# microsoft/vision-longformer

Measured on NVIDIA H100. Metric: images/sec ViL-Small 224x224 training, higher is better.
Workload: dtype bf16

## Files before the change

### vision_longformer_b200/csrc/vil_common.cuh

```cuda
#pragma once
#include <cuda_runtime.h>
#include <cuda_bf16.h>
#include <cuda_fp16.h>
#include <stdint.h>
#include "../../include/vil_attn.h"

namespace vil {

struct Geo {
  int B, H, D;
  int nx, ny, w, g, exact, mode;
  int padx, pady, mx, my;
  int Nloc, N, w2;
  int npc;
  int noffs;
  int offR[9], offC[9];
  int has_bias;
  float scale;
  float drop_p, drop_scale;
  uint32_t drop_thresh;
  uint32_t seed_lo, seed_hi, drop_off;
};

inline long long ws_off_delta_g(const Geo& g) { return ((long long)g.B * g.H * g.Nloc + 63) & ~63LL; }
// ... 80 lines not shown
}
__device__ __forceinline__ uint32_t philox_word(const uint4& x, uint32_t w) {
  return w == 0 ? x.x : w == 1 ? x.y : w == 2 ? x.z : x.w;
}
__device__ __forceinline__ bool drop_keep(const Geo& g, uint32_t row, uint32_t col, uint32_t sid) {
  return philox_word(philox(g, col >> 2, row, sid), col & 3) >= g.drop_thresh;
}
__device__ __forceinline__ void drop_keep2(const Geo& g, uint32_t row, uint32_t col, uint32_t sid, bool& k0, bool& k1) {
  const uint4 x = philox(g, col >> 2, row, sid);
  const uint32_t w = col & 3;
  k0 = philox_word(x, w) >= g.drop_thresh;
  const uint32_t u1 = w == 3 ? philox(g, (col >> 2) + 1, row, sid).x : philox_word(x, w + 1);
  k1 = u1 >= g.drop_thresh;
}

__device__ __forceinline__ float warp_sum(float v) {
#pragma unroll
  for (int o = 16; o > 0; o >>= 1) v += __shfl_xor_sync(0xffffffffu, v, o);
  return v;
}

}
```

### vision_longformer_b200/csrc/vil_epilogue.cuh

```cuda
#pragma once
#include "vil_common.cuh"

namespace vil {
namespace epi {

constexpr int kWarps = 4;
constexpr int kAnThreads = kWarps * 32;
constexpr int kThreads = 256;

template <typename T> struct Vec4;
template <> struct Vec4<float> {
  static __device__ __forceinline__ void ld(const float* p, float (&r)[4]) {
    const float4 v = __ldg(reinterpret_cast<const float4*>(p)); r[0] = v.x; r[1] = v.y; r[2] = v.z; r[3] = v.w;
  }
  static __device__ __forceinline__ void st(float* p, const float (&r)[4]) {
    *reinterpret_cast<float4*>(p) = make_float4(r[0], r[1], r[2], r[3]);
  }
};
template <> struct Vec4<__nv_bfloat16> {
  static __device__ __forceinline__ void ld(const __nv_bfloat16* p, float (&r)[4]) {
    const uint2 raw = __ldg(reinterpret_cast<const uint2*>(p));
    const float2 a = __bfloat1622float2(*reinterpret_cast<const __nv_bfloat162*>(&raw.x));
    const float2 b = __bfloat1622float2(*reinterpret_cast<const __nv_bfloat162*>(&raw.y));
    r[0] = a.x; r[1] = a.y; r[2] = b.x; r[3] = b.y;
// ... 237 lines not shown
  float t = 0.f;
  if (col < K * C)
    for (int p = py; p < nparts; p += 8) t += partial[(long long)p * K * C + col];
  sm[py][threadIdx.x & 31] = t;
  __syncthreads();
  if (py == 0 && col < K * C) {
    float r = 0.f;
#pragma unroll
    for (int k = 0; k < 8; ++k) r += sm[k][threadIdx.x & 31];
    const int seg = col / C;
    float* o = seg == 0 ? o0 : (seg == 1 ? o1 : o2);
    if (o != nullptr) o[col - seg * C] = r;
  }
}

__device__ __forceinline__ float ex2_approx(float x) { float y; asm("ex2.approx.ftz.f32 %0, %1;" : "=f"(y) : "f"(x)); return y; }
__device__ __forceinline__ float rcp_approx(float x) { float y; asm("rcp.approx.ftz.f32 %0, %1;" : "=f"(y) : "f"(x)); return y; }
struct GeluTerms { float half_erfc_neg; float gauss; };
__device__ __forceinline__ GeluTerms gelu_terms(float u) {
  const float ax = fabsf(u) * 0.70710678118654752f;
  const float e = ex2_approx(-0.72134752044448170f * u * u);
  const float t = rcp_approx(fmaf(0.3275911f, ax, 1.f));
  float pl = fmaf(1.061405429f, t, -1.453152027f);
  pl = fmaf(pl, t, 1.421413741f);
  pl = fmaf(pl, t, -0.284496736f);
  pl = fmaf(pl, t, 0.254829592f);
  const float q = 0.5f * pl * t * e;
  GeluTerms r;
  r.half_erfc_neg = u >= 0.f ? 1.f - q : q;
  r.gauss = e;
  return r;
// ... 134 lines not shown
```

### vision_longformer_b200/csrc/vil_simt.cuh

```cuda
#pragma once
#include "vil_common.cuh"

namespace vil {

template <int HD> struct Tile {
  static constexpr int HH = HD / 2;
  static constexpr int HS = HD + 8;
  static __device__ __forceinline__ int off(int half) { return half * (HH + 4); }
};

struct ChunkId { int b, h, R, C, piece; };

__device__ __forceinline__ ChunkId decode_block(const Geo& g, int bid) {
  ChunkId c;
  c.piece = bid % g.npc; bid /= g.npc;
  c.C = bid % g.my; bid /= g.my;
  c.R = bid % g.mx; bid /= g.mx;
  c.h = bid % g.H;
  c.b = bid / g.H;
  return c;
}

template <typename T, int HD, bool DROP = false>
__global__ void __launch_bounds__(128)
// ... 90 lines not shown
      sp += __shfl_xor_sync(0xffffffffu, sp, 1);
      float bias = 0.f; bool ok = qvalid;
      if (f == 2) {
        if (geo.has_bias) bias = g2l[((long long)geo.H + h) * geo.g + kvr[j]];
      } else {
        const int dr = qr - kvr[j], dc = qc - kvc[j];
        if (geo.exact == 1 && (abs(dr) > w || abs(dc) > w)) ok = false;
        if (geo.has_bias && ok) bias = tab[(dr + 2 * w - 1) * tw + dc + 2 * w - 1];
      }
      if (ok) {
        const float s = fmaf(geo.scale, sp, bias);
        const float* vd = Vs + j * HS + TL::off(half);
        if constexpr (DROP) {
          const float km = drop_keep(geo, drow, (uint32_t)(cbase + j), dsid) ? 1.f : 0.f;
          if (s > m) {
            const float corr = __expf(m - s);
            lsum = lsum * corr + 1.f;
#pragma unroll
            for (int i = 0; i < HH; ++i) oh[i] = fmaf(oh[i], corr, km * vd[i]);
            m = s;
          } else {
            const float p = __expf(s - m);
            lsum += p;
#pragma unroll
            for (int i = 0; i < HH; ++i) oh[i] = fmaf(p * km, vd[i], oh[i]);
          }
        } else {
          if (s > m) {
            const float corr = __expf(m - s);
            lsum = lsum * corr + 1.f;
#pragma unroll
            for (int i = 0; i < HH; ++i) oh[i] = fmaf(oh[i], corr, vd[i]);
            m = s;
          } else {
            const float p = __expf(s - m);
            lsum += p;
#pragma unroll
            for (int i = 0; i < HH; ++i) oh[i] = fmaf(p, vd[i], oh[i]);
          }
        }
      }
    }
  }
  if (qvalid) {
    const float inv = (lsum > 0.f ? 1.f / lsum : 0.f) * (DROP ? geo.drop_scale : 1.f);
#pragma unroll
    for (int i = 0; i < HH; ++i) oh[i] *= inv;
    const long long tokq = (long long)r * geo.ny + c;
    store_seg<T, HH>(row_ptr_w<T>(o, b, h, tokq), half * HH, D, oh);
    if (half == 0) lse[((long long)b * geo.H + h) * geo.Nloc + tokq] = m + logf(lsum);
// ... 38 lines not shown
  for (int i = 0; i < 8; ++i) oacc[i] = 0.f;
  const float bl = geo.has_bias ? g2l[(long long)h * geo.g + a] : 0.f;
  for (int base = row0 + warp * RPW; base < row1; base += ROWS) {
    const int j = base + rw;
    const bool valid = j < row1;
    const int jc = valid ? j : row1 - 1;
    float kk[8], vv[8];
    load_seg<T, 8>(row_ptr<T>(kg, b, h, jc), 8 * sub, D, kk);
    load_seg<T, 8>(row_ptr<T>(vg, b, h, jc), 8 * sub, D, vv);
    const float sp = group_sum<LPR>(dot8(q8, kk));
    float bias = bl;
    if (geo.has_bias && jc < geo.g) bias = g2g[((long long)h * geo.g + a) * geo.g + jc];
    const float sc = valid ? fmaf(geo.scale, sp, bias) : -INFINITY;
    const float mn = fmaxf(m, sc);
    if (mn > -INFINITY) {
      const float corr = __expf(m - mn), p = __expf(sc - mn);
      lsum = fmaf(lsum, corr, p);
      float pk = p;
      if constexpr (DROP) {
        if (!drop_keep(geo, (uint32_t)a, (uint32_t)j, 2u * (uint32_t)(b * geo.H + h) + 1u)) pk = 0.f;
      }
#pragma unroll
      for (int i = 0; i < 8; ++i) oacc[i] = fmaf(oacc[i], corr, pk * vv[i]);
      m = mn;
    }
  }
  float mw = m;
#pragma unroll
  for (int o = LPR; o < 32; o <<= 1) mw = fmaxf(mw, __shfl_xor_sync(0xffffffffu, mw, o));
  const float scw = (m == -INFINITY) ? 0.f : __expf(m - mw);
  const float lw = rows_sum<LPR>(lsum * scw);
#pragma unroll
  for (int i = 0; i < 8; ++i) {
    const float x = rows_sum<LPR>(oacc[i] * scw);
    if (rw == 0) red_o[warp][8 * sub + i] = x;
  }
  if (lane == 0) { red_m[warp] = mw; red_l[warp] = lw; }
  __syncthreads();
  if (tid < HD) {
    float M = -INFINITY;
    for (int x = 0; x < 8; ++x) M = fmaxf(M, red_m[x]);
    float L = 0.f, O = 0.f;
    for (int x = 0; x < 8; ++x) {
      const float s2 = (red_m[x] == -INFINITY) ? 0.f : __expf(red_m[x] - M);
      L += red_l[x] * s2; O += red_o[x][tid] * s2;
    }
    if (tid < D) row_ptr_w<TO>(og, b, h, a)[tid] = ElemTraits<TO>::from_f(DROP ? O / L * geo.drop_scale : O / L);
    if (tid == 0) lse_g[((long long)b * geo.H + h) * geo.g + a] = M + logf(L);
  }
}

template <typename T, typename TO = T>
__global__ void simt_bwd_delta(Geo geo, T4 o, T4 d_o, T4 og, T4 d_og,
                               float* __restrict__ delta, float* __restrict__ delta_g) {
  const long long rows_loc = (long long)geo.B * geo.H * geo.Nloc;
  const long long rows = rows_loc + (long long)geo.B * geo.H * geo.g;
  const long long idx = (long long)blockIdx.x * (blockDim.x >> 2) + (threadIdx.x >> 2);
  const int sub = threadIdx.x & 3;
  float acc = 0.f;
// ... 120 lines not shown
      const float* vd = Vs + j * HS + TL::off(half);
      float sp = 0.f, dpp = 0.f;
#pragma unroll
      for (int i = 0; i < HH; ++i) { sp = fmaf(qh[i], kd[i], sp); dpp = fmaf(doh[i], vd[i], dpp); }
      sp += __shfl_xor_sync(0xffffffffu, sp, 1);
      dpp += __shfl_xor_sync(0xffffffffu, dpp, 1);
      float bias = 0.f; bool ok = qvalid; int bidx = -1;
      if (f == 2) {
        if (geo.has_bias) bias = g2l[((long long)geo.H + h) * geo.g + kvr[j]];
      } else {
        const int dr = qr - kvr[j], dc = qc - kvc[j];
        if (geo.exact == 1 && (abs(dr) > w || abs(dc) > w)) ok = false;
        if (geo.has_bias && ok) { bidx = (dr + 2 * w - 1) * tw + dc + 2 * w - 1; bias = tab[bidx]; }
      }
      if (ok) {
        const float p = __expf(fmaf(geo.scale, sp, bias) - lse_i);
        if constexpr (DROP) dpp *= km;
        const float ds = p * (dpp - del_i);
#pragma unroll
        for (int i = 0; i < HH; ++i) dqh[i] = fmaf(ds, kd[i], dqh[i]);
        if (bidx >= 0 && half == 0 && d_table != nullptr)
          atomicAdd(d_table + (long long)bidx * geo.H + h, ds);
      }
    }
  }
  if (qvalid) {
#pragma unroll
    for (int i = 0; i < HH; ++i) dqh[i] *= geo.scale;
    store_seg<T, HH>(row_ptr_w<T>(dq, b, h, tokq), half * HH, D, dqh);
  }
}
// ... 76 lines not shown
      __syncthreads();
      for (int i2 = 0; i2 < 64; ++i2) {
        if (!qfl[i2]) continue;
        const float* qd = Qs + i2 * HS + TL::off(half);
        const float* gd = Gs + i2 * HS + TL::off(half);
        float sp = 0.f, dpp = 0.f;
#pragma unroll
        for (int i = 0; i < HH; ++i) { sp = fmaf(kh[i], qd[i], sp); dpp = fmaf(vh[i], gd[i], dpp); }
        sp += __shfl_xor_sync(0xffffffffu, sp, 1);
        dpp += __shfl_xor_sync(0xffffffffu, dpp, 1);
        const int dr = qrs[i2] - vr, dc = qcs[i2] - vc;
        bool ok = kvis;
        if (geo.exact == 1 && (abs(dr) > w || abs(dc) > w)) ok = false;
        if (ok) {
          const float bias = geo.has_bias ? tab[(dr + 2 * w - 1) * tw + dc + 2 * w - 1] : 0.f;
          float p = __expf(fmaf(geo.scale, sp, bias) - lse_s[i2]);
          if constexpr (DROP) {
            const float km = drop_keep(geo, (uint32_t)qtok[i2], (uint32_t)(geo.g + oi * geo.w2 + lk), 2u * (uint32_t)(b * geo.H + h))
                                 ? geo.drop_scale : 0.f;
            const float ds = p * (dpp * km - del_s[i2]);
            p *= km;
#pragma unroll
            for (int i = 0; i < HH; ++i) { dkh[i] = fmaf(ds, qd[i], dkh[i]); dvh[i] = fmaf(p, gd[i], dvh[i]); }
          } else {
            const float ds = p * (dpp - del_s[i2]);
#pragma unroll
            for (int i = 0; i < HH; ++i) { dkh[i] = fmaf(ds, qd[i], dkh[i]); dvh[i] = fmaf(p, gd[i], dvh[i]); }
          }
        }
      }
    }
// ... 33 lines not shown
  load_seg<T, 8>(row_ptr<T>(v, b, h, t), 8 * sub, D, v8);
  const float bias = geo.has_bias ? g2l[((long long)geo.H + h) * geo.g + t] : 0.f;
  float adk[8], adv[8], adb = 0.f;
#pragma unroll
  for (int i = 0; i < 8; ++i) { adk[i] = 0.f; adv[i] = 0.f; }
  const long long base_l = ((long long)b * geo.H + h) * geo.Nloc;
  for (int base = row0 + warp * RPW; base < row1; base += ROWS) {
    const int i2 = base + rw;
    const bool valid = i2 < row1;
    const int ic = valid ? i2 : row1 - 1;
    float qq[8], gg[8];
    load_seg<T, 8>(row_ptr<T>(q, b, h, ic), 8 * sub, D, qq);
    load_seg<T, 8>(row_ptr<T>(d_o, b, h, ic), 8 * sub, D, gg);
    const float ls = lse[base_l + ic], dl = delta[base_l + ic];
    const float sp = group_sum<LPR>(dot8(qq, k8)), dpp = group_sum<LPR>(dot8(gg, v8));
    float p = valid ? __expf(fmaf(geo.scale, sp, bias) - ls) : 0.f;
    float dpk = dpp;
    if constexpr (DROP) {
      const float km = drop_keep(geo, (uint32_t)ic, (uint32_t)t, 2u * (uint32_t)(b * geo.H + h)) ? geo.drop_scale : 0.f;
      dpk = dpp * km;
      const float ds = p * (dpk - dl);
      if (sub == 0) adb += ds;
      p *= km;
#pragma unroll
      for (int i = 0; i < 8; ++i) { adk[i] = fmaf(ds, qq[i], adk[i]); adv[i] = fmaf(p, gg[i], adv[i]); }
    } else {
      const float ds = p * (dpk - dl);
      if (sub == 0) adb += ds;
#pragma unroll
      for (int i = 0; i < 8; ++i) { adk[i] = fmaf(ds, qq[i], adk[i]); adv[i] = fmaf(p, gg[i], adv[i]); }
    }
// ... 44 lines not shown
      const int jc = valid ? j : row1 - 1;
      float kk[8], vv[8], ok_[8], ov_[8];
      load_seg<T, 8>(row_ptr<T>(kg, b, h, jc), 8 * sub, D, kk);
      load_seg<T, 8>(row_ptr<T>(vg, b, h, jc), 8 * sub, D, vv);
      const bool rmw = base < rmw_rows;
      if (add && rmw) {
        load_seg<TO, 8>(row_ptr<TO>(dkg, b, h, jc), 8 * sub, D, ok_);
        load_seg<TO, 8>(row_ptr<TO>(dvg, b, h, jc), 8 * sub, D, ov_);
      } else {
#pragma unroll
        for (int i = 0; i < 8; ++i) { ok_[i] = 0.f; ov_[i] = 0.f; }
      }
      const float sp = group_sum<LPR>(dot8(q8, kk)), dpp = group_sum<LPR>(dot8(g8, vv));
      float bias = bl;
      if (geo.has_bias && jc < geo.g) bias = g2g[((long long)h * geo.g + a) * geo.g + jc];
      const float p = valid ? __expf(fmaf(geo.scale, sp, bias) - lg) : 0.f;
      float km = 1.f;
      if constexpr (DROP) km = drop_keep(geo, (uint32_t)a, (uint32_t)jc, 2u * (uint32_t)(b * geo.H + h) + 1u) ? geo.drop_scale : 0.f;
      const float ds = DROP ? p * (dpp * km - dg) : p * (dpp - dg);
      const float pv = DROP ? p * km : p;
      if (geo.has_bias && valid && sub == 0) {
        if (j < geo.g) { if (d_g2g) atomicAdd(d_g2g + ((long long)h * geo.g + a) * geo.g + j, ds); }
        else adb += ds;
      }
      const float dss = ds * geo.scale;
#pragma unroll
      for (int i = 0; i < 8; ++i) {
        adq[i] = fmaf(ds, kk[i], adq[i]);
        ok_[i] = fmaf(dss, q8[i], ok_[i]);
        ov_[i] = fmaf(pv, g8[i], ov_[i]);
      }
// ... 46 lines not shown
```

### vision_longformer_b200/csrc/vil_wgmma.cuh

```cuda
#pragma once
#include "vil_common.cuh"
#include "vil_sm90.cuh"

namespace vil {
namespace wg {

constexpr int kThreads = 128;

struct Cta { int b, h, R, C, piece; };

__device__ __forceinline__ Cta decode(const Geo& g, int bid) {
  Cta c;
  c.piece = bid % g.npc; bid /= g.npc;
  c.C = bid % g.my; bid /= g.my;
  c.R = bid % g.mx; bid /= g.mx;
  c.h = bid % g.H;
  c.b = bid / g.H;
  return c;
}

__device__ __forceinline__ int acc_row(int i) { return ((threadIdx.x >> 5) << 4) + ((threadIdx.x & 31) >> 2) + (((i >> 1) & 1) << 3); }
__device__ __forceinline__ int acc_col(int i) { return ((i >> 2) << 3) + ((threadIdx.x & 3) << 1) + (i & 1); }

constexpr int kStages = 3;
// ... 43 lines not shown
}

__device__ __forceinline__ void drop_rows(const Geo& geo, int R, int C, int piece, uint32_t (&row)[2]) {
#pragma unroll
  for (int e = 0; e < 2; ++e) {
    const int l = piece * 64 + acc_row(2 * e);
    row[e] = (uint32_t)((R * geo.w + l / geo.w) * geo.ny + C * geo.w + l % geo.w);
  }
}

struct Visit {
  int r, c;
  int dR, dC;
  int cut;
  int oi;
};

__device__ __forceinline__ int visit_list(const Geo& geo, int R, int C, int sgn, Visit* vl) {
  int n = 0;
  for (int oi = 0; oi < geo.noffs; ++oi) {
    const int dR = geo.offR[oi], dC = geo.offC[oi];
    int r = R + sgn * dR, c = C + sgn * dC;
    if (geo.exact == -1) { r = (r + geo.mx) % geo.mx; c = (c + geo.my) % geo.my; }
    else if (r < 0 || r >= geo.mx || c < 0 || c >= geo.my) continue;
    const int qR = sgn > 0 ? R : r, qC = sgn > 0 ? C : c;
    if (threadIdx.x == 0) vl[n] = Visit{r, c, dR, dC, (qR + dR == geo.mx - 1) | ((qC + dC == geo.my - 1) << 1), oi};
    ++n;
  }
  return n;
}

__device__ __forceinline__ int drop_col_base(const Geo& geo, const Visit* vl, int ngp, int pi) {
  if (pi < ngp) return pi * 64;
  const int vi = (pi - ngp) / geo.npc;
  return geo.g + vl[vi].oi * geo.w2 + (pi - ngp - vi * geo.npc) * 64;
}

struct SlotWalk {
  int vi, pj, kr, kc;
  int r0, c0, dr, dc;
  __device__ __forceinline__ SlotWalk(const Geo& geo, int slot)
      : vi(0), pj(0), r0(slot / geo.w), c0(slot % geo.w), dr(64 / geo.w), dc(64 % geo.w) { kr = r0; kc = c0; }
  __device__ __forceinline__ void next(const Geo& geo) {
    if (++pj == geo.npc) { pj = 0; ++vi; kr = r0; kc = c0; return; }
    kr += dr; kc += dc;
    if (kc >= geo.w) { kc -= geo.w; ++kr; }
  }
};

__device__ __forceinline__ void chunk_key(const Geo& geo, const Visit& v, int kr, int kc, long long& tok, bool& ok, int& vr, int& vc) {
  const int w = geo.w;
  const int ar = v.r * w + kr, ac = v.c * w + kc;
  const bool real = (ar < geo.nx) && (ac < geo.ny);
  if (geo.exact == -1)
    ok = !(((v.cut & 1) && (kr >= w - geo.padx)) || ((v.cut & 2) && (kc >= w - geo.pady)));
  else
    ok = real;
  tok = (ok && real) ? geo.g + (long long)ar * geo.ny + ac : -1;
  vr = v.dR * w + kr; vc = v.dC * w + kc;
}

__device__ __forceinline__ void key_slot(const Geo& geo, const Visit* vl, int ngp, int pi, int slot, SlotWalk& wk, int& gk,
                                         long long& tok, bool& ok, int& vr, int& vc) {
  gk = -1; tok = -1; ok = false; vr = 0; vc = 0;
  if (pi < ngp) {
    const int t = pi * 64 + slot;
    if (t < geo.g) { gk = t; tok = t; ok = true; }
    return;
  }
  if (wk.kr < geo.w) chunk_key(geo, vl[wk.vi], wk.kr, wk.kc, tok, ok, vr, vc);
  wk.next(geo);
}

struct KeyCols {
  float* bias;
  int* tix;
  short* kr;
  short* kc;
};
struct QRows {
  int qr[2], qc[2];
  bool ok[2];
};

__device__ __forceinline__ QRows query_rows(const Geo& geo, int R, int C, int piece) {
// ... 3 lines not shown
  for (int e = 0; e < 2; ++e) {
    const int l = piece * 64 + acc_row(2 * e);
    const bool in = l < geo.w2;
    q.qr[e] = in ? l / w : 0; q.qc[e] = in ? l % w : 0;
    q.ok[e] = in && (R * w + q.qr[e] < geo.nx) && (C * w + q.qc[e] < geo.ny);
  }
  return q;
}

__device__ __forceinline__ void stage_key_cols(const Geo& geo, const KeyCols& kc, int h, const float* __restrict__ g2l, int gk,
                                               bool ok, int vr, int vc) {
  const int slot = threadIdx.x >> 1;
  float bias = ok ? 0.f : -INFINITY;
  if (gk >= 0 && geo.has_bias) bias = g2l[((long long)geo.H + h) * geo.g + gk];
  kc.bias[slot] = bias;
  kc.tix[slot] = vr * (4 * geo.w - 1) + vc;
  kc.kr[slot] = (short)vr;
  kc.kc[slot] = (short)vc;
}

__device__ __forceinline__ void row_tix(const Geo& geo, const QRows& q, int (&tb)[2]) {
  const int w = geo.w, tw = 4 * w - 1;
  tb[0] = (q.qr[0] + 2 * w - 1) * tw + q.qc[0] + 2 * w - 1;
  tb[1] = (q.qr[1] + 2 * w - 1) * tw + q.qc[1] + 2 * w - 1;
}

template <bool RPE, bool WIN>
__device__ __forceinline__ float key_score(const Geo& geo, const KeyCols& kc, const float* tab, const QRows& q, const int (&tb)[2],
                                           int e, int j, int gl, float s, int& bidx) {
  float bias = kc.bias[j];
  bidx = -1;
  if (RPE && j >= gl) { bidx = tb[e] - kc.tix[j]; bias += tab[bidx]; }
  if (WIN && (abs(q.qr[e] - kc.kr[j]) > geo.w || abs(q.qc[e] - kc.kc[j]) > geo.w)) return -INFINITY;
// ... 15 lines not shown
    mx[e] = fmaxf(mx[e], s[i]);
  }
}

template <bool RPE, bool WIN>
__device__ __forceinline__ void dq_scores(float (&s)[32], const float (&dp)[32], const Geo& geo, const KeyCols& kc,
                                          const float* tab, const QRows& q, int gl, const float (&lse_r)[2],
                                          const float (&del_r)[2], float* __restrict__ d_table, int h) {
  int tb[2] = {0, 0};
  if (RPE) row_tix(geo, q, tb);
#pragma unroll
  for (int i = 0; i < 32; ++i) {
    const int e = (i >> 1) & 1;
    int bidx;
    const float val = key_score<RPE, WIN>(geo, kc, tab, q, tb, e, acc_col(i), gl, s[i], bidx);
    const float ds = __expf(val - lse_r[e]) * (dp[i] - del_r[e]);
    if (RPE && d_table != nullptr && bidx >= 0 && q.ok[e] && val != -INFINITY)
      atomicAdd(d_table + (long long)bidx * geo.H + h, ds);
    s[i] = ds;
  }
}

constexpr size_t kKeyCols = 64 * (4 + 4 + 2 + 2);
constexpr size_t kQueryCols = 64 * (4 + 4 + 4 + 2 + 2 + 1);
constexpr size_t kVisits = 9 * sizeof(Visit);
__host__ __device__ constexpr size_t query_cols_bytes(bool drop) { return kQueryCols + (drop ? 64 * sizeof(int) : 0); }

__device__ __forceinline__ KeyCols key_cols(unsigned char* meta, int stage) {
  KeyCols kc;
  kc.bias = reinterpret_cast<float*>(meta + stage * kKeyCols);
  kc.tix = reinterpret_cast<int*>(kc.bias + 64);
// ... 6 lines not shown
  static constexpr size_t tiles = (1 + 2 * kStages) * 64 * HD * 2;
  static size_t total(int tabn) { return (tiles + kStages * kKeyCols + kVisits + (size_t)tabn * 4 + 15) & ~size_t(15); }
};
template <int HD> struct DqSmem {
  static constexpr size_t tiles = (2 + 2 * kStages) * 64 * HD * 2;
  static size_t total(int tabn) { return (tiles + kStages * kKeyCols + kVisits + (size_t)tabn * 4 + 15) & ~size_t(15); }
};
template <int HD> struct DkvSmem {
  static constexpr size_t tiles = (2 + 2 * kStages) * 64 * HD * 2;
  static size_t total(int tabn, bool drop = false) {
    return (tiles + kStages * query_cols_bytes(drop) + kVisits + 64 * sizeof(int) + (size_t)tabn * 4 + 15) & ~size_t(15);
  }
};

template <typename T, int HD>
__device__ __forceinline__ void issue_key_piece(const Geo& geo, int pi, int npieces, int ngp, const Visit* vl, SlotWalk& wk,
                                                T* ring, unsigned char* meta, const T* kb, long long kst, const T* vb,
                                                long long vst, int h, const float* __restrict__ g2l) {
  if (pi < npieces) {
    const int slot = threadIdx.x >> 1, half = threadIdx.x & 1, st = pi % kStages;
    int gk, vr, vc;
    long long tok;
    bool ok;
    key_slot(geo, vl, ngp, pi, slot, wk, gk, tok, ok, vr, vc);
    T* Ks = ring + st * 2 * 64 * HD;
    stage_row<T, HD>(Ks, kb, kst, tok, slot, half, geo.D);
    stage_row<T, HD>(Ks + 64 * HD, vb, vst, tok, slot, half, geo.D);
    if (half == 0) stage_key_cols(geo, key_cols(meta, st), h, g2l, gk, ok, vr, vc);
  }
  sm90::cp_async_commit();
}

__device__ __forceinline__ void ring_wait() {
  sm90::cp_async_wait<kStages - 2>();
  sm90::fence_proxy_async();
  __syncthreads();
}

template <typename T, int HD, typename TO, bool DROP = false>
__global__ void __launch_bounds__(kThreads, HD <= 32 ? 5 : 3)
wg_fwd_local(Geo geo, T4 q, T4 k, T4 v, T4 o, float* __restrict__ lse, const float* __restrict__ table,
             const float* __restrict__ g2l) {
  constexpr int HH = HD / 2, TILE = 64 * HD;
  using W64 = sm90::Wg<T, 64>;
  using WHD = sm90::Wg<T, HD>;
  extern __shared__ __align__(128) unsigned char smem_raw[];
  T* Qs = reinterpret_cast<T*>(smem_raw);
  T* ring = Qs + TILE;
  unsigned char* meta = reinterpret_cast<unsigned char*>(ring + 2 * kStages * TILE);
  Visit* vl = reinterpret_cast<Visit*>(meta + kStages * kKeyCols);
  float* tab = reinterpret_cast<float*>(vl + 9);
  const int tabn = geo.has_bias ? (4 * geo.w - 1) * (4 * geo.w - 1) : 0;

  const Cta cid = decode(geo, blockIdx.x);
  const int b = cid.b, h = cid.h, R = cid.R, C = cid.C;
// ... 3 lines not shown
  {
    const int l = cid.piece * 64 + slot;
    const int r = R * w + l / w, c = C * w + l % w;
    const bool real = l < geo.w2 && r < geo.nx && c < geo.ny;
    stage_row<T, HD>(Qs, row_ptr<T>(q, b, h, 0), q.st, real ? (long long)r * geo.ny + c : -1, slot, half, D);
  }
  float m[2] = {-INFINITY, -INFINITY}, lsum[2] = {0.f, 0.f};
  float oacc[HH];
#pragma unroll
  for (int i = 0; i < HH; ++i) oacc[i] = 0.f;

  const int ngp = (geo.g + 63) / 64, npieces = ngp + visit_list(geo, R, C, 1, vl) * geo.npc;
  const int epi = key_epilogue(geo);
  const T* kb = row_ptr<T>(k, b, h, 0);
  const T* vb = row_ptr<T>(v, b, h, 0);
  SlotWalk wk(geo, slot);
  __syncthreads();
#pragma unroll
  for (int p = 0; p < kStages - 1; ++p)
    issue_key_piece<T, HD>(geo, p, npieces, ngp, vl, wk, ring, meta, kb, k.st, vb, v.st, h, g2l);
  for (int pi = 0; pi < npieces; ++pi) {
    ring_wait();
    issue_key_piece<T, HD>(geo, pi + kStages - 1, npieces, ngp, vl, wk, ring, meta, kb, k.st, vb, v.st, h, g2l);
    const int st = pi % kStages;
    const T* Ks = ring + st * 2 * TILE;
    const T* Vs = Ks + TILE;
    const KeyCols kcol = key_cols(meta, st);
    float s[32];
    sm90::wg_fence();
#pragma unroll
    for (int kk = 0; kk < HD / 16; ++kk) W64::ss(s, sm90::desc(Qs, HD, kk), sm90::desc(Ks, HD, kk), kk > 0);
    sm90::wg_commit();
    sm90::wg_wait0();
    sm90::reg_fence(s);
    float mx[2] = {-INFINITY, -INFINITY};
    const int gl = geo.g - pi * 64;
    switch (epi) {
      case 0: fwd_scores<false, false>(s, mx, geo, kcol, tab, query_rows(geo, R, C, cid.piece), gl); break;
      case 1: fwd_scores<false, true>(s, mx, geo, kcol, tab, query_rows(geo, R, C, cid.piece), gl); break;
      case 2: fwd_scores<true, false>(s, mx, geo, kcol, tab, query_rows(geo, R, C, cid.piece), gl); break;
      default: fwd_scores<true, true>(s, mx, geo, kcol, tab, query_rows(geo, R, C, cid.piece), gl); break;
    }
    float corr[2];
#pragma unroll
    for (int e = 0; e < 2; ++e) {
      mx[e] = fmaxf(mx[e], __shfl_xor_sync(0xffffffffu, mx[e], 1));
      mx[e] = fmaxf(mx[e], __shfl_xor_sync(0xffffffffu, mx[e], 2));
      const float mn = fmaxf(m[e], mx[e]);
      corr[e] = (mn == -INFINITY) ? 1.f : __expf(m[e] - mn);
      m[e] = mn;
      lsum[e] *= corr[e];
    }
#pragma unroll
    for (int i = 0; i < 32; ++i) {
      const int e = (i >> 1) & 1;
      const float p = (m[e] == -INFINITY) ? 0.f : __expf(s[i] - m[e]);
      s[i] = p;
      lsum[e] += p;
    }
#pragma unroll
    for (int i = 0; i < HH; ++i) oacc[i] *= corr[(i >> 1) & 1];
    if constexpr (DROP) {
      uint32_t drow[2];
      drop_rows(geo, R, C, cid.piece, drow);
      drop_key_piece(s, geo, drow, drop_col_base(geo, vl, ngp, pi), 2u * (uint32_t)(b * geo.H + h), 1.f);
    }
    uint32_t a[4][4];
#pragma unroll
    for (int kk = 0; kk < 4; ++kk) to_a_frag<T>(s, kk, a[kk]);
    sm90::wg_fence();
#pragma unroll
    for (int kk = 0; kk < 4; ++kk) WHD::rs(oacc, a[kk], sm90::desc_mn(Vs, HD, kk), 1);
    sm90::wg_commit();
    sm90::wg_wait0();
    sm90::reg_fence(oacc);
  }
  const QRows qrow = query_rows(geo, R, C, cid.piece);
#pragma unroll
  for (int e = 0; e < 2; ++e) {
    lsum[e] += __shfl_xor_sync(0xffffffffu, lsum[e], 1);
    lsum[e] += __shfl_xor_sync(0xffffffffu, lsum[e], 2);
    if (!qrow.ok[e]) continue;
    const long long tokq = (long long)(R * w + qrow.qr[e]) * geo.ny + (C * w + qrow.qc[e]);
    const float inv = lsum[e] > 0.f ? 1.f / lsum[e] : 0.f;
// ... 38 lines not shown
    lse_r[e] = INFINITY; del_r[e] = 0.f;
    if (qrow.ok[e]) {
      const long long tokq = (long long)(R * w + qrow.qr[e]) * geo.ny + (C * w + qrow.qc[e]);
      lse_r[e] = lse[bh * geo.Nloc + tokq];
      del_r[e] = delta[bh * geo.Nloc + tokq];
    }
  }
  float dqacc[HH];
#pragma unroll
  for (int i = 0; i < HH; ++i) dqacc[i] = 0.f;

  const int ngp = (geo.g + 63) / 64, npieces = ngp + visit_list(geo, R, C, 1, vl) * geo.npc;
  const int epi = key_epilogue(geo);
  const T* kb = row_ptr<T>(k, b, h, 0);
  const T* vb = row_ptr<T>(v, b, h, 0);
  SlotWalk wk(geo, slot);
  __syncthreads();
#pragma unroll
  for (int p = 0; p < kStages - 1; ++p)
    issue_key_piece<T, HD>(geo, p, npieces, ngp, vl, wk, ring, meta, kb, k.st, vb, v.st, h, g2l);
  for (int pi = 0; pi < npieces; ++pi) {
    ring_wait();
    issue_key_piece<T, HD>(geo, pi + kStages - 1, npieces, ngp, vl, wk, ring, meta, kb, k.st, vb, v.st, h, g2l);
    const int st = pi % kStages;
    const T* Ks = ring + st * 2 * TILE;
    const T* Vs = Ks + TILE;
    const KeyCols kcol = key_cols(meta, st);
    float s[32], dp[32];
    sm90::wg_fence();
#pragma unroll
    for (int kk = 0; kk < HD / 16; ++kk) W64::ss(s, sm90::desc(Qs, HD, kk), sm90::desc(Ks, HD, kk), kk > 0);
#pragma unroll
    for (int kk = 0; kk < HD / 16; ++kk) W64::ss(dp, sm90::desc(Gs, HD, kk), sm90::desc(Vs, HD, kk), kk > 0);
    sm90::wg_commit();
    sm90::wg_wait0();
    sm90::reg_fence(s);
    sm90::reg_fence(dp);
    const int gl = geo.g - pi * 64;
// ... 63 lines not shown
}

__device__ __forceinline__ QueryCols query_cols(unsigned char* meta, int stage, int bytes) {
  QueryCols qc;
  qc.lse = reinterpret_cast<float*>(meta + stage * bytes);
  qc.del = qc.lse + 64;
  qc.tix = reinterpret_cast<int*>(qc.del + 64);
  qc.qr = reinterpret_cast<short*>(qc.tix + 64);
  qc.qc = qc.qr + 64;
  qc.cut = reinterpret_cast<unsigned char*>(qc.qc + 64);
  qc.tok = reinterpret_cast<int*>(qc.cut + 64);
  return qc;
}

template <typename T, int HD, bool DROP>
__device__ __forceinline__ void issue_query_piece(const Geo& geo, int qp, int npieces, const Visit* vl, SlotWalk& wk, T* ring,
                                                  unsigned char* meta, const T* qb, long long qst, const T* gb, long long gst,
                                                  const float* __restrict__ lse, const float* __restrict__ delta) {
  if (qp < npieces) {
    const int slot = threadIdx.x >> 1, half = threadIdx.x & 1, st = qp % kStages, w = geo.w;
    bool qv = false;
    long long tq = 0;
    int qa = 0, qb2 = 0, cut = 0;
    if (wk.kr < w) {
      const Visit vq = vl[wk.vi];
      const int r = vq.r * w + wk.kr, c = vq.c * w + wk.kc;
      qv = (r < geo.nx) && (c < geo.ny);
      tq = (long long)r * geo.ny + c;
      qa = wk.kr - vq.dR * w; qb2 = wk.kc - vq.dC * w; cut = vq.cut;
    }
    wk.next(geo);
    T* Qs = ring + st * 2 * 64 * HD;
    stage_row<T, HD>(Qs, qb, qst, qv ? tq : -1, slot, half, geo.D);
    stage_row<T, HD>(Qs + 64 * HD, gb, gst, qv ? tq : -1, slot, half, geo.D);
    if (half == 0) {
      const QueryCols qcol = query_cols(meta, st, (int)query_cols_bytes(DROP));
      if (qv) {
        sm90::cp_async4(qcol.lse + slot, lse + tq);
        sm90::cp_async4(qcol.del + slot, delta + tq);
      } else {
        qcol.lse[slot] = INFINITY;
        qcol.del[slot] = 0.f;
      }
      const int tw = 4 * w - 1;
      qcol.tix[slot] = qa * tw + qb2;
      qcol.qr[slot] = (short)qa; qcol.qc[slot] = (short)qb2;
      qcol.cut[slot] = (unsigned char)cut;
      if (DROP) qcol.tok[slot] = (int)tq;
    }
  }
  sm90::cp_async_commit();
}

__device__ __forceinline__ int query_epilogue(const Geo& geo) {
  return (geo.has_bias ? 3 : 0) + (geo.exact == 1 ? 1 : geo.exact == -1 ? 2 : 0);
}

template <bool RPE, int MASK>
__device__ __forceinline__ void dkv_probs(float (&s)[32], float (&dp)[32], const Geo& geo, const QueryCols& qc, const float* tab,
                                          const KRows& kr) {
#pragma unroll
  for (int i = 0; i < 32; ++i) {
    const int e = (i >> 1) & 1, j = acc_col(i);
    float x = fmaf(geo.scale, s[i], RPE ? tab[qc.tix[j] - kr.tb[e]] : 0.f) - qc.lse[j];
    if (MASK == 1 && (abs(qc.qr[j] - kr.kr[e]) > geo.w || abs(qc.qc[j] - kr.kc[e]) > geo.w)) x = -INFINITY;
    if (MASK == 2 && (qc.cut[j] & kr.cut[e])) x = -INFINITY;
    const float p = __expf(x);
    s[i] = p;
    dp[i] = p * (dp[i] - qc.del[j]);
  }
}

template <typename T, int HD, typename TO, bool DROP = false>
__global__ void __launch_bounds__(kThreads, (HD <= 32 ? 4 : 3) - (DROP ? 1 : 0))
wg_bwd_dkv(Geo geo, T4 q, T4 k, T4 v, T4 d_o, T4 dk, T4 dv, const float* __restrict__ lse, const float* __restrict__ delta,
           const float* __restrict__ table) {
  constexpr int HH = HD / 2, TILE = 64 * HD;
  using W64 = sm90::Wg<T, 64>;
  using WHD = sm90::Wg<T, HD>;
  extern __shared__ __align__(128) unsigned char smem_raw[];
  T* Ks = reinterpret_cast<T*>(smem_raw);
  T* Vs = Ks + TILE;
// ... 14 lines not shown
  for (int i = tid; i < tabn; i += kThreads) tab[i] = table[(long long)i * geo.H + h];
  {
    const int lk = cid.piece * 64 + slot;
    const int ar = KR * w + lk / w, ac = KC * w + lk % w;
    const long long tokk = (lk < geo.w2 && ar < geo.nx && ac < geo.ny) ? geo.g + (long long)ar * geo.ny + ac : -1;
    stage_row<T, HD>(Ks, row_ptr<T>(k, b, h, 0), k.st, tokk, slot, half, D);
    stage_row<T, HD>(Vs, row_ptr<T>(v, b, h, 0), v.st, tokk, slot, half, D);
    if (half == 0) kpos[slot] = key_pos(geo, cid.piece, slot);
  }
  float dkacc[HH], dvacc[HH];
#pragma unroll
  for (int i = 0; i < HH; ++i) { dkacc[i] = 0.f; dvacc[i] = 0.f; }

  const int npieces = visit_list(geo, KR, KC, -1, vl) * geo.npc;
  const int epi = query_epilogue(geo);
  SlotWalk wk(geo, slot);
  __syncthreads();
#pragma unroll
  for (int p = 0; p < kStages - 1; ++p)
    issue_query_piece<T, HD, DROP>(geo, p, npieces, vl, wk, ring, meta, row_ptr<T>(q, b, h, 0), q.st,
                                   row_ptr<T>(d_o, b, h, 0), d_o.st, lse + bh * geo.Nloc, delta + bh * geo.Nloc);
  for (int qp = 0; qp < npieces; ++qp) {
    ring_wait();
    issue_query_piece<T, HD, DROP>(geo, qp + kStages - 1, npieces, vl, wk, ring, meta, row_ptr<T>(q, b, h, 0), q.st,
                                   row_ptr<T>(d_o, b, h, 0), d_o.st, lse + bh * geo.Nloc, delta + bh * geo.Nloc);
    const int st = qp % kStages;
    const T* Qs = ring + st * 2 * TILE;
    const T* Gs = Qs + TILE;
    const QueryCols qcol = query_cols(meta, st, cols);
    uint32_t keep = 0;
    if constexpr (DROP) {
      const int vi = qp / geo.npc;
      const uint32_t c0 = (uint32_t)(geo.g + vl[vi].oi * geo.w2 + cid.piece * 64), sid = 2u * (uint32_t)(b * geo.H + h);
#pragma unroll 1
      for (int i = 0; i < 32; ++i)
        keep |= (uint32_t)drop_keep(geo, (uint32_t)qcol.tok[acc_col(i)], c0 + (uint32_t)acc_row(i), sid) << i;
    }
    float s[32], dp[32];
    sm90::wg_fence();
// ... 50 lines not shown
```

Before: 3782.

## Use ex2-based fast exp, precompute visit limits, and pack softmax probs directly

Replaces __expf with an ex2.approx-based fast_exp across the SIMT and wgmma attention kernels. It also precomputes per-visit token bases and bound limits so key and query slot walking needs less per-piece index arithmetic, and skips bias/mask metadata writes when they are unused. In the non-dropout forward path the probabilities are packed straight into A fragments, and the occupancy hint for the small-head forward kernel is raised. The fast exp uses an approximate ex2 with flush-to-zero, and the packed bit-field limits assume window sizes below 256.

Result: faster. 3883, median of 6 (+2.7%).

```diff
diff --git a/vision_longformer_b200/csrc/vil_common.cuh b/vision_longformer_b200/csrc/vil_common.cuh
--- a/vision_longformer_b200/csrc/vil_common.cuh
+++ b/vision_longformer_b200/csrc/vil_common.cuh
@@ -118,6 +118,9 @@
   k1 = u1 >= g.drop_thresh;
 }
 
+__device__ __forceinline__ float ex2_approx(float x) { float y; asm("ex2.approx.ftz.f32 %0, %1;" : "=f"(y) : "f"(x)); return y; }
+__device__ __forceinline__ float fast_exp(float x) { return ex2_approx(x * 1.4426950216293334961f); }
+
 __device__ __forceinline__ float warp_sum(float v) {
 #pragma unroll
   for (int o = 16; o > 0; o >>= 1) v += __shfl_xor_sync(0xffffffffu, v, o);
diff --git a/vision_longformer_b200/csrc/vil_epilogue.cuh b/vision_longformer_b200/csrc/vil_epilogue.cuh
--- a/vision_longformer_b200/csrc/vil_epilogue.cuh
+++ b/vision_longformer_b200/csrc/vil_epilogue.cuh
@@ -275,7 +275,6 @@
   }
 }
 
-__device__ __forceinline__ float ex2_approx(float x) { float y; asm("ex2.approx.ftz.f32 %0, %1;" : "=f"(y) : "f"(x)); return y; }
 __device__ __forceinline__ float rcp_approx(float x) { float y; asm("rcp.approx.ftz.f32 %0, %1;" : "=f"(y) : "f"(x)); return y; }
 struct GeluTerms { float half_erfc_neg; float gauss; };
 __device__ __forceinline__ GeluTerms gelu_terms(float u) {
diff --git a/vision_longformer_b200/csrc/vil_simt.cuh b/vision_longformer_b200/csrc/vil_simt.cuh
--- a/vision_longformer_b200/csrc/vil_simt.cuh
+++ b/vision_longformer_b200/csrc/vil_simt.cuh
@@ -128,26 +128,26 @@
         if constexpr (DROP) {
           const float km = drop_keep(geo, drow, (uint32_t)(cbase + j), dsid) ? 1.f : 0.f;
           if (s > m) {
-            const float corr = __expf(m - s);
+            const float corr = fast_exp(m - s);
             lsum = lsum * corr + 1.f;
 #pragma unroll
             for (int i = 0; i < HH; ++i) oh[i] = fmaf(oh[i], corr, km * vd[i]);
             m = s;
           } else {
-            const float p = __expf(s - m);
+            const float p = fast_exp(s - m);
             lsum += p;
 #pragma unroll
             for (int i = 0; i < HH; ++i) oh[i] = fmaf(p * km, vd[i], oh[i]);
           }
         } else {
           if (s > m) {
-            const float corr = __expf(m - s);
+            const float corr = fast_exp(m - s);
             lsum = lsum * corr + 1.f;
 #pragma unroll
             for (int i = 0; i < HH; ++i) oh[i] = fmaf(oh[i], corr, vd[i]);
             m = s;
           } else {
-            const float p = __expf(s - m);
+            const float p = fast_exp(s - m);
             lsum += p;
 #pragma unroll
             for (int i = 0; i < HH; ++i) oh[i] = fmaf(p, vd[i], oh[i]);
@@ -216,7 +216,7 @@
     const float sc = valid ? fmaf(geo.scale, sp, bias) : -INFINITY;
     const float mn = fmaxf(m, sc);
     if (mn > -INFINITY) {
-      const float corr = __expf(m - mn), p = __expf(sc - mn);
+      const float corr = fast_exp(m - mn), p = fast_exp(sc - mn);
       lsum = fmaf(lsum, corr, p);
       float pk = p;
       if constexpr (DROP) {
@@ -230,7 +230,7 @@
   float mw = m;
 #pragma unroll
   for (int o = LPR; o < 32; o <<= 1) mw = fmaxf(mw, __shfl_xor_sync(0xffffffffu, mw, o));
-  const float scw = (m == -INFINITY) ? 0.f : __expf(m - mw);
+  const float scw = (m == -INFINITY) ? 0.f : fast_exp(m - mw);
   const float lw = rows_sum<LPR>(lsum * scw);
 #pragma unroll
   for (int i = 0; i < 8; ++i) {
@@ -244,7 +244,7 @@
     for (int x = 0; x < 8; ++x) M = fmaxf(M, red_m[x]);
     float L = 0.f, O = 0.f;
     for (int x = 0; x < 8; ++x) {
-      const float s2 = (red_m[x] == -INFINITY) ? 0.f : __expf(red_m[x] - M);
+      const float s2 = (red_m[x] == -INFINITY) ? 0.f : fast_exp(red_m[x] - M);
       L += red_l[x] * s2; O += red_o[x][tid] * s2;
     }
     if (tid < D) row_ptr_w<TO>(og, b, h, a)[tid] = ElemTraits<TO>::from_f(DROP ? O / L * geo.drop_scale : O / L);
@@ -395,7 +395,7 @@
         if (geo.has_bias && ok) { bidx = (dr + 2 * w - 1) * tw + dc + 2 * w - 1; bias = tab[bidx]; }
       }
       if (ok) {
-        const float p = __expf(fmaf(geo.scale, sp, bias) - lse_i);
+        const float p = fast_exp(fmaf(geo.scale, sp, bias) - lse_i);
         if constexpr (DROP) dpp *= km;
         const float ds = p * (dpp - del_i);
 #pragma unroll
@@ -502,7 +502,7 @@
         if (geo.exact == 1 && (abs(dr) > w || abs(dc) > w)) ok = false;
         if (ok) {
           const float bias = geo.has_bias ? tab[(dr + 2 * w - 1) * tw + dc + 2 * w - 1] : 0.f;
-          float p = __expf(fmaf(geo.scale, sp, bias) - lse_s[i2]);
+          float p = fast_exp(fmaf(geo.scale, sp, bias) - lse_s[i2]);
           if constexpr (DROP) {
             const float km = drop_keep(geo, (uint32_t)qtok[i2], (uint32_t)(geo.g + oi * geo.w2 + lk), 2u * (uint32_t)(b * geo.H + h))
                                  ? geo.drop_scale : 0.f;
@@ -566,7 +566,7 @@
     load_seg<T, 8>(row_ptr<T>(d_o, b, h, ic), 8 * sub, D, gg);
     const float ls = lse[base_l + ic], dl = delta[base_l + ic];
     const float sp = group_sum<LPR>(dot8(qq, k8)), dpp = group_sum<LPR>(dot8(gg, v8));
-    float p = valid ? __expf(fmaf(geo.scale, sp, bias) - ls) : 0.f;
+    float p = valid ? fast_exp(fmaf(geo.scale, sp, bias) - ls) : 0.f;
     float dpk = dpp;
     if constexpr (DROP) {
       const float km = drop_keep(geo, (uint32_t)ic, (uint32_t)t, 2u * (uint32_t)(b * geo.H + h)) ? geo.drop_scale : 0.f;
@@ -641,7 +641,7 @@
       const float sp = group_sum<LPR>(dot8(q8, kk)), dpp = group_sum<LPR>(dot8(g8, vv));
       float bias = bl;
       if (geo.has_bias && jc < geo.g) bias = g2g[((long long)h * geo.g + a) * geo.g + jc];
-      const float p = valid ? __expf(fmaf(geo.scale, sp, bias) - lg) : 0.f;
+      const float p = valid ? fast_exp(fmaf(geo.scale, sp, bias) - lg) : 0.f;
       float km = 1.f;
       if constexpr (DROP) km = drop_keep(geo, (uint32_t)a, (uint32_t)jc, 2u * (uint32_t)(b * geo.H + h) + 1u) ? geo.drop_scale : 0.f;
       const float ds = DROP ? p * (dpp * km - dg) : p * (dpp - dg);
diff --git a/vision_longformer_b200/csrc/vil_wgmma.cuh b/vision_longformer_b200/csrc/vil_wgmma.cuh
--- a/vision_longformer_b200/csrc/vil_wgmma.cuh
+++ b/vision_longformer_b200/csrc/vil_wgmma.cuh
@@ -81,9 +81,12 @@
   int dR, dC;
   int cut;
   int oi;
+  int tok0;
+  int lim;
 };
 
 __device__ __forceinline__ int visit_list(const Geo& geo, int R, int C, int sgn, Visit* vl) {
+  const int w = geo.w;
   int n = 0;
   for (int oi = 0; oi < geo.noffs; ++oi) {
     const int dR = geo.offR[oi], dC = geo.offC[oi];
@@ -91,7 +94,17 @@
     if (geo.exact == -1) { r = (r + geo.mx) % geo.mx; c = (c + geo.my) % geo.my; }
     else if (r < 0 || r >= geo.mx || c < 0 || c >= geo.my) continue;
     const int qR = sgn > 0 ? R : r, qC = sgn > 0 ? C : c;
-    if (threadIdx.x == 0) vl[n] = Visit{r, c, dR, dC, (qR + dR == geo.mx - 1) | ((qC + dC == geo.my - 1) << 1), oi};
+    if (threadIdx.x == 0) {
+      const int cut = (qR + dR == geo.mx - 1) | ((qC + dC == geo.my - 1) << 1);
+      const int nr = min(w, geo.nx - r * w), nc = min(w, geo.ny - c * w);
+      int lim = nr | nc << 8;
+      if (sgn > 0) {
+        const int okr = geo.exact != -1 ? nr : (cut & 1) ? w - geo.padx : w;
+        const int okc = geo.exact != -1 ? nc : (cut & 2) ? w - geo.pady : w;
+        lim = min(nr, okr) | min(nc, okc) << 8 | okr << 16 | okc << 24;
+      }
+      vl[n] = Visit{r, c, dR, dC, cut, oi, r * w * geo.ny + c * w, lim};
+    }
     ++n;
   }
   return n;
@@ -103,39 +116,35 @@
   return geo.g + vl[vi].oi * geo.w2 + (pi - ngp - vi * geo.npc) * 64;
 }
 
-struct SlotWalk {
-  int vi, pj, kr, kc;
-  int r0, c0, dr, dc;
-  __device__ __forceinline__ SlotWalk(const Geo& geo, int slot)
-      : vi(0), pj(0), r0(slot / geo.w), c0(slot % geo.w), dr(64 / geo.w), dc(64 % geo.w) { kr = r0; kc = c0; }
+struct PieceWalk {
+  int vi = 0, pj = 0, qa = 0, ra = 0;
   __device__ __forceinline__ void next(const Geo& geo) {
-    if (++pj == geo.npc) { pj = 0; ++vi; kr = r0; kc = c0; return; }
-    kr += dr; kc += dc;
+    if (++pj == geo.npc) { pj = 0; ++vi; qa = 0; ra = 0; return; }
+    qa += 64 / geo.w; ra += 64 % geo.w;
+    if (ra >= geo.w) { ra -= geo.w; ++qa; }
+  }
+  __device__ __forceinline__ void pos(const Geo& geo, int so, int& kr, int& kc) const {
+    kr = qa + (so & 0xff); kc = ra + (so >> 8);
     if (kc >= geo.w) { kc -= geo.w; ++kr; }
   }
 };
-
-__device__ __forceinline__ void chunk_key(const Geo& geo, const Visit& v, int kr, int kc, long long& tok, bool& ok, int& vr, int& vc) {
-  const int w = geo.w;
-  const int ar = v.r * w + kr, ac = v.c * w + kc;
-  const bool real = (ar < geo.nx) && (ac < geo.ny);
-  if (geo.exact == -1)
-    ok = !(((v.cut & 1) && (kr >= w - geo.padx)) || ((v.cut & 2) && (kc >= w - geo.pady)));
-  else
-    ok = real;
-  tok = (ok && real) ? geo.g + (long long)ar * geo.ny + ac : -1;
-  vr = v.dR * w + kr; vc = v.dC * w + kc;
-}
-
-__device__ __forceinline__ void key_slot(const Geo& geo, const Visit* vl, int ngp, int pi, int slot, SlotWalk& wk, int& gk,
-                                         long long& tok, bool& ok, int& vr, int& vc) {
+__device__ __forceinline__ int slot_offset(const Geo& geo, int slot) { return slot / geo.w | (slot % geo.w) << 8; }
+
+__device__ __forceinline__ void key_slot(const Geo& geo, const Visit* vl, int ngp, int pi, int slot, int so, PieceWalk& wk,
+                                         int& gk, long long& tok, bool& ok, int& vr, int& vc) {
   gk = -1; tok = -1; ok = false; vr = 0; vc = 0;
   if (pi < ngp) {
     const int t = pi * 64 + slot;
     if (t < geo.g) { gk = t; tok = t; ok = true; }
     return;
   }
-  if (wk.kr < geo.w) chunk_key(geo, vl[wk.vi], wk.kr, wk.kc, tok, ok, vr, vc);
+  int kr, kc;
+  wk.pos(geo, so, kr, kc);
+  const Visit* v = vl + wk.vi;
+  const int lim = v->lim;
+  ok = kr < ((lim >> 16) & 0xff) && kc < (lim >> 24);
+  if (kr < (lim & 0xff) && kc < ((lim >> 8) & 0xff)) tok = geo.g + v->tok0 + kr * geo.ny + kc;
+  if ((geo.has_bias || geo.exact == 1) && kr < geo.w) { vr = v->dR * geo.w + kr; vc = v->dC * geo.w + kc; }
   wk.next(geo);
 }
 
@@ -169,9 +178,11 @@
   float bias = ok ? 0.f : -INFINITY;
   if (gk >= 0 && geo.has_bias) bias = g2l[((long long)geo.H + h) * geo.g + gk];
   kc.bias[slot] = bias;
-  kc.tix[slot] = vr * (4 * geo.w - 1) + vc;
-  kc.kr[slot] = (short)vr;
-  kc.kc[slot] = (short)vc;
+  if (geo.has_bias || geo.exact == 1) {
+    kc.tix[slot] = vr * (4 * geo.w - 1) + vc;
+    kc.kr[slot] = (short)vr;
+    kc.kc[slot] = (short)vc;
+  }
 }
 
 __device__ __forceinline__ void row_tix(const Geo& geo, const QRows& q, int (&tb)[2]) {
@@ -217,7 +228,7 @@
     const int e = (i >> 1) & 1;
     int bidx;
     const float val = key_score<RPE, WIN>(geo, kc, tab, q, tb, e, acc_col(i), gl, s[i], bidx);
-    const float ds = __expf(val - lse_r[e]) * (dp[i] - del_r[e]);
+    const float ds = fast_exp(val - lse_r[e]) * (dp[i] - del_r[e]);
     if (RPE && d_table != nullptr && bidx >= 0 && q.ok[e] && val != -INFINITY)
       atomicAdd(d_table + (long long)bidx * geo.H + h, ds);
     s[i] = ds;
@@ -254,15 +265,15 @@
 };
 
 template <typename T, int HD>
-__device__ __forceinline__ void issue_key_piece(const Geo& geo, int pi, int npieces, int ngp, const Visit* vl, SlotWalk& wk,
-                                                T* ring, unsigned char* meta, const T* kb, long long kst, const T* vb,
-                                                long long vst, int h, const float* __restrict__ g2l) {
+__device__ __forceinline__ void issue_key_piece(const Geo& geo, int pi, int npieces, int ngp, const Visit* vl, int so,
+                                                PieceWalk& wk, T* ring, unsigned char* meta, const T* kb, long long kst,
+                                                const T* vb, long long vst, int h, const float* __restrict__ g2l) {
   if (pi < npieces) {
     const int slot = threadIdx.x >> 1, half = threadIdx.x & 1, st = pi % kStages;
     int gk, vr, vc;
     long long tok;
     bool ok;
-    key_slot(geo, vl, ngp, pi, slot, wk, gk, tok, ok, vr, vc);
+    key_slot(geo, vl, ngp, pi, slot, so, wk, gk, tok, ok, vr, vc);
     T* Ks = ring + st * 2 * 64 * HD;
     stage_row<T, HD>(Ks, kb, kst, tok, slot, half, geo.D);
     stage_row<T, HD>(Ks + 64 * HD, vb, vst, tok, slot, half, geo.D);
@@ -278,7 +289,7 @@
 }
 
 template <typename T, int HD, typename TO, bool DROP = false>
-__global__ void __launch_bounds__(kThreads, HD <= 32 ? 5 : 3)
+__global__ void __launch_bounds__(kThreads, HD <= 32 ? (DROP ? 5 : 6) : 3)
 wg_fwd_local(Geo geo, T4 q, T4 k, T4 v, T4 o, float* __restrict__ lse, const float* __restrict__ table,
              const float* __restrict__ g2l) {
   constexpr int HH = HD / 2, TILE = 64 * HD;
@@ -312,14 +323,15 @@
   const int epi = key_epilogue(geo);
   const T* kb = row_ptr<T>(k, b, h, 0);
   const T* vb = row_ptr<T>(v, b, h, 0);
-  SlotWalk wk(geo, slot);
+  const int so = slot_offset(geo, slot);
+  PieceWalk wk;
   __syncthreads();
 #pragma unroll
   for (int p = 0; p < kStages - 1; ++p)
-    issue_key_piece<T, HD>(geo, p, npieces, ngp, vl, wk, ring, meta, kb, k.st, vb, v.st, h, g2l);
+    issue_key_piece<T, HD>(geo, p, npieces, ngp, vl, so, wk, ring, meta, kb, k.st, vb, v.st, h, g2l);
   for (int pi = 0; pi < npieces; ++pi) {
     ring_wait();
-    issue_key_piece<T, HD>(geo, pi + kStages - 1, npieces, ngp, vl, wk, ring, meta, kb, k.st, vb, v.st, h, g2l);
+    issue_key_piece<T, HD>(geo, pi + kStages - 1, npieces, ngp, vl, so, wk, ring, meta, kb, k.st, vb, v.st, h, g2l);
     const int st = pi % kStages;
     const T* Ks = ring + st * 2 * TILE;
     const T* Vs = Ks + TILE;
@@ -345,16 +357,20 @@
       mx[e] = fmaxf(mx[e], __shfl_xor_sync(0xffffffffu, mx[e], 1));
       mx[e] = fmaxf(mx[e], __shfl_xor_sync(0xffffffffu, mx[e], 2));
       const float mn = fmaxf(m[e], mx[e]);
-      corr[e] = (mn == -INFINITY) ? 1.f : __expf(m[e] - mn);
+      corr[e] = (mn == -INFINITY) ? 1.f : fast_exp(m[e] - mn);
       m[e] = mn;
       lsum[e] *= corr[e];
     }
-#pragma unroll
-    for (int i = 0; i < 32; ++i) {
+    uint32_t a[4][4];
+#pragma unroll
+    for (int i = 0; i < 32; i += 2) {
       const int e = (i >> 1) & 1;
-      const float p = (m[e] == -INFINITY) ? 0.f : __expf(s[i] - m[e]);
-      s[i] = p;
-      lsum[e] += p;
+      const float p0 = (m[e] == -INFINITY) ? 0.f : fast_exp(s[i] - m[e]);
+      const float p1 = (m[e] == -INFINITY) ? 0.f : fast_exp(s[i + 1] - m[e]);
+      lsum[e] += p0;
+      lsum[e] += p1;
+      if constexpr (DROP) { s[i] = p0; s[i + 1] = p1; }
+      else a[i >> 3][(i >> 1) & 3] = sm90::pack2<T>(p0, p1);
     }
 #pragma unroll
     for (int i = 0; i < HH; ++i) oacc[i] *= corr[(i >> 1) & 1];
@@ -362,10 +378,9 @@
       uint32_t drow[2];
       drop_rows(geo, R, C, cid.piece, drow);
       drop_key_piece(s, geo, drow, drop_col_base(geo, vl, ngp, pi), 2u * (uint32_t)(b * geo.H + h), 1.f);
-    }
-    uint32_t a[4][4];
-#pragma unroll
-    for (int kk = 0; kk < 4; ++kk) to_a_frag<T>(s, kk, a[kk]);
+#pragma unroll
+      for (int kk = 0; kk < 4; ++kk) to_a_frag<T>(s, kk, a[kk]);
+    }
     sm90::wg_fence();
 #pragma unroll
     for (int kk = 0; kk < 4; ++kk) WHD::rs(oacc, a[kk], sm90::desc_mn(Vs, HD, kk), 1);
@@ -434,14 +449,15 @@
   const int epi = key_epilogue(geo);
   const T* kb = row_ptr<T>(k, b, h, 0);
   const T* vb = row_ptr<T>(v, b, h, 0);
-  SlotWalk wk(geo, slot);
+  const int so = slot_offset(geo, slot);
+  PieceWalk wk;
   __syncthreads();
 #pragma unroll
   for (int p = 0; p < kStages - 1; ++p)
-    issue_key_piece<T, HD>(geo, p, npieces, ngp, vl, wk, ring, meta, kb, k.st, vb, v.st, h, g2l);
+    issue_key_piece<T, HD>(geo, p, npieces, ngp, vl, so, wk, ring, meta, kb, k.st, vb, v.st, h, g2l);
   for (int pi = 0; pi < npieces; ++pi) {
     ring_wait();
-    issue_key_piece<T, HD>(geo, pi + kStages - 1, npieces, ngp, vl, wk, ring, meta, kb, k.st, vb, v.st, h, g2l);
+    issue_key_piece<T, HD>(geo, pi + kStages - 1, npieces, ngp, vl, so, wk, ring, meta, kb, k.st, vb, v.st, h, g2l);
     const int st = pi % kStages;
     const T* Ks = ring + st * 2 * TILE;
     const T* Vs = Ks + TILE;
@@ -535,20 +551,21 @@
 }
 
 template <typename T, int HD, bool DROP>
-__device__ __forceinline__ void issue_query_piece(const Geo& geo, int qp, int npieces, const Visit* vl, SlotWalk& wk, T* ring,
-                                                  unsigned char* meta, const T* qb, long long qst, const T* gb, long long gst,
-                                                  const float* __restrict__ lse, const float* __restrict__ delta) {
+__device__ __forceinline__ void issue_query_piece(const Geo& geo, int qp, int npieces, const Visit* vl, int so, PieceWalk& wk,
+                                                  T* ring, unsigned char* meta, const T* qb, long long qst, const T* gb,
+                                                  long long gst, const float* __restrict__ lse, const float* __restrict__ delta) {
   if (qp < npieces) {
     const int slot = threadIdx.x >> 1, half = threadIdx.x & 1, st = qp % kStages, w = geo.w;
     bool qv = false;
-    long long tq = 0;
-    int qa = 0, qb2 = 0, cut = 0;
-    if (wk.kr < w) {
-      const Visit vq = vl[wk.vi];
-      const int r = vq.r * w + wk.kr, c = vq.c * w + wk.kc;
-      qv = (r < geo.nx) && (c < geo.ny);
-      tq = (long long)r * geo.ny + c;
-      qa = wk.kr - vq.dR * w; qb2 = wk.kc - vq.dC * w; cut = vq.cut;
+    int tq = 0, qa = 0, qb2 = 0, cut = 0;
+    int kr, kc;
+    wk.pos(geo, so, kr, kc);
+    if (kr < w) {
+      const Visit* vq = vl + wk.vi;
+      const int lim = vq->lim;
+      qv = kr < (lim & 0xff) && kc < ((lim >> 8) & 0xff);
+      tq = vq->tok0 + kr * geo.ny + kc;
+      if (geo.has_bias || geo.exact != 0) { qa = kr - vq->dR * w; qb2 = kc - vq->dC * w; cut = vq->cut; }
     }
     wk.next(geo);
     T* Qs = ring + st * 2 * 64 * HD;
@@ -563,11 +580,12 @@
         qcol.lse[slot] = INFINITY;
         qcol.del[slot] = 0.f;
       }
-      const int tw = 4 * w - 1;
-      qcol.tix[slot] = qa * tw + qb2;
-      qcol.qr[slot] = (short)qa; qcol.qc[slot] = (short)qb2;
-      qcol.cut[slot] = (unsigned char)cut;
-      if (DROP) qcol.tok[slot] = (int)tq;
+      if (geo.has_bias || geo.exact != 0) {
+        qcol.tix[slot] = qa * (4 * w - 1) + qb2;
+        qcol.qr[slot] = (short)qa; qcol.qc[slot] = (short)qb2;
+        qcol.cut[slot] = (unsigned char)cut;
+      }
+      if (DROP) qcol.tok[slot] = tq;
     }
   }
   sm90::cp_async_commit();
@@ -586,7 +604,7 @@
     float x = fmaf(geo.scale, s[i], RPE ? tab[qc.tix[j] - kr.tb[e]] : 0.f) - qc.lse[j];
     if (MASK == 1 && (abs(qc.qr[j] - kr.kr[e]) > geo.w || abs(qc.qc[j] - kr.kc[e]) > geo.w)) x = -INFINITY;
     if (MASK == 2 && (qc.cut[j] & kr.cut[e])) x = -INFINITY;
-    const float p = __expf(x);
+    const float p = fast_exp(x);
     s[i] = p;
     dp[i] = p * (dp[i] - qc.del[j]);
   }
@@ -631,15 +649,16 @@
 
   const int npieces = visit_list(geo, KR, KC, -1, vl) * geo.npc;
   const int epi = query_epilogue(geo);
-  SlotWalk wk(geo, slot);
+  const int so = slot_offset(geo, slot);
+  PieceWalk wk;
   __syncthreads();
 #pragma unroll
   for (int p = 0; p < kStages - 1; ++p)
-    issue_query_piece<T, HD, DROP>(geo, p, npieces, vl, wk, ring, meta, row_ptr<T>(q, b, h, 0), q.st,
+    issue_query_piece<T, HD, DROP>(geo, p, npieces, vl, so, wk, ring, meta, row_ptr<T>(q, b, h, 0), q.st,
                                    row_ptr<T>(d_o, b, h, 0), d_o.st, lse + bh * geo.Nloc, delta + bh * geo.Nloc);
   for (int qp = 0; qp < npieces; ++qp) {
     ring_wait();
-    issue_query_piece<T, HD, DROP>(geo, qp + kStages - 1, npieces, vl, wk, ring, meta, row_ptr<T>(q, b, h, 0), q.st,
+    issue_query_piece<T, HD, DROP>(geo, qp + kStages - 1, npieces, vl, so, wk, ring, meta, row_ptr<T>(q, b, h, 0), q.st,
                                    row_ptr<T>(d_o, b, h, 0), d_o.st, lse + bh * geo.Nloc, delta + bh * geo.Nloc);
     const int st = qp % kStages;
     const T* Qs = ring + st * 2 * TILE;
```
